# succinctlabs/tendermintx

Hardware: AMD Instinct MI355X
Metric: skip-circuit witness-gen ms at VALIDATOR_SET_SIZE_MAX=128 (lower is better)
Workload: dtype int64; 1 GPU; SkipCircuit VALIDATOR_SET_SIZE_MAX=128, batch of 256 proofs over 1 GPU(s) (BASELINE configs[3] batch per GPU, weak-scaled), 100 validators in 128 lanes, 4 distinct validator set(s) per batch, 90% sign; n_max=128, proofs_total=256, proofs_per_gpu=256, workload_name=survey8d, parallelism=proof-sharded x1, no data-path collective

## Files before the change

### include/tmx.h

```cpp
#ifndef TMX_H
#define TMX_H
#include <stddef.h>
#include <stdint.h>

#ifdef __cplusplus
extern "C" {
#endif

#define TMX_KIND_SKIP 0
#define TMX_KIND_STEP 1

#define TMX_N_MAX_LIMIT 512

#define TMX_VALIDATOR_MESSAGE_BYTES_LENGTH_MAX 124
#define TMX_VALIDATOR_BYTE_LENGTH_MAX 46
#define TMX_PROTOBUF_CHAIN_ID_SIZE_BYTES 52
#define TMX_HEADER_PROOF_DEPTH 4

#define TMX_FLAG_SIGNED 1u
#define TMX_FLAG_PRESENT 2u

typedef enum {
  TMX_OK = 0,
  TMX_ERR_BAD_ARG = -1,
// ... 235 lines not shown
int32_t tmx_finish_batch_device(tmx_ctx* ctx, int32_t kind, uint32_t n_proofs, const void* d_proofs, const void* d_targets,
                                const void* d_trusteds, const void* d_ed, void* d_out_elems, void* d_reports, void* hip_stream);
int32_t tmx_last_kernel_ms(tmx_ctx* ctx, float ms[TMX_N_KERNELS]);
int32_t tmx_kernel_ms_mean(tmx_ctx* ctx, uint32_t last_k, float ms[TMX_N_KERNELS]);
int32_t tmx_sync(tmx_ctx* ctx);
int32_t tmx_last_dedup(tmx_ctx* ctx, uint32_t* n_unique, uint32_t* used_tables);
enum tmx_proof_path {
  TMX_PROOF_PATH_NONE = 0,
  TMX_PROOF_PATH_TINY = 1,
  TMX_PROOF_PATH_ROLES = 2,
  TMX_PROOF_PATH_R168 = 3,
  TMX_PROOF_PATH_K256 = 4,
  TMX_PROOF_PATH_WIDE = 5
};
int32_t tmx_last_proof_path(tmx_ctx* ctx);

#define TMX_UNIQUE_ID_BYTES 128
void tmx_shard_range(uint64_t n_items, uint32_t rank, uint32_t world, uint64_t* lo, uint64_t* hi);
int32_t tmx_comm_unique_id(uint8_t out[TMX_UNIQUE_ID_BYTES]);
int32_t tmx_comm_create(tmx_ctx* ctx, const uint8_t unique_id[TMX_UNIQUE_ID_BYTES] , uint32_t rank, uint32_t world);
int32_t tmx_comm_destroy(tmx_ctx* ctx);
int32_t tmx_comm_info(const tmx_ctx* ctx, uint32_t* rank, uint32_t* world);
int32_t tmx_comm_abort(tmx_ctx* ctx);
int32_t tmx_comm_sync(tmx_ctx* ctx, void* hip_stream, uint32_t timeout_ms);
int32_t tmx_witness_batch_sharded_device(tmx_ctx* ctx, int32_t kind, uint32_t n_total, const void* d_proofs, const void* d_targets,
                                         const void* d_trusteds, void* d_out_elems, void* d_reports, uint32_t gather, void* hip_stream);
int32_t tmx_witness_validator_sharded_device(tmx_ctx* ctx, int32_t kind, uint32_t n_proofs, const void* d_proofs, const void* d_targets,
                                             const void* d_trusteds, void* d_out_elems, void* d_reports, void* hip_stream);

int32_t tmx_trace_rows_sharded_device(tmx_ctx* ctx, int32_t kind, uint32_t n_total, const void* d_targets, const void* d_trusteds, void* d_trace_out,
// ... 264 lines not shown
```

### tendermintx_amd/_lib.py

```python
import ctypes as C
import ctypes.util
import importlib.util
import os
import sys

_HERE = os.path.dirname(os.path.abspath(__file__))
LIB_PATH = os.environ.get("TMX_LIB") or os.path.join(_HERE, "libtmx.so")

KIND_SKIP, KIND_STEP = 0, 1
FLAG_SIGNED, FLAG_PRESENT = 1, 2
N_KERNELS = 4
KERNEL_NAMES = ("k_eddsa", "k_proof", "k_verdict", "k_serialize")
ED_STRIDE = 448
SEC_HINT, SEC_DERIVED, SEC_ALL = 1, 2, 3
PROOF_PATH_NONE, PROOF_PATH_TINY, PROOF_PATH_ROLES, PROOF_PATH_R168, PROOF_PATH_K256, PROOF_PATH_WIDE = range(6)
TRACE_LADDERS, TRACE_SHA512, TRACE_SHA256, TRACE_MATCH, TRACE_TREE, TRACE_HEADER, TRACE_ALL = 1, 2, 4, 8, 16, 32, 63
TRACE_LADDERS_QUOTIENT = 64
AIR_SHA256_HELPER_COLS, AIR_SHA256_CONSTRAINTS = 300, 315
TRACE_SHA256_HELPER, TRACE_SHA256_QUOTIENT = 128, 256
AIR_SHA256_SCHED_HELPER_COLS, AIR_SHA256_SCHED_CONSTRAINTS = 115, 117
TRACE_SHA256_SCHED_HELPER, TRACE_SHA256_SCHED_QUOTIENT = 512, 1024
AIR_SHA256_INIT_HELPER_COLS, AIR_SHA256_INIT_CONSTRAINTS = 315, 337
TRACE_SHA256_INIT_HELPER, TRACE_SHA256_INIT_QUOTIENT = 2048, 4096
TRACE_SHA256_LINK_HELPER, TRACE_SHA256_LINK_QUOTIENT = 8192, 16384
AIR_SHA256_PUBLIC_WIDTH, AIR_SHA256_LINK_HELPER_COLS, AIR_SHA256_LINK_CONSTRAINTS = 26, 33, 50


class ValidatorRec(C.Structure):
    _fields_ = [("pubkey", C.c_uint8 * 32), ("signature", C.c_uint8 * 64), ("message", C.c_uint8 * 124),
                ("message_byte_length", C.c_uint16), ("validator_byte_length", C.c_uint8), ("flags", C.c_uint8),
# ... 375 lines not shown
    L.tmx_witness_batch_sharded_device.argtypes = [C.c_void_p, C.c_int32, C.c_uint32, C.c_void_p, C.c_void_p, C.c_void_p, C.c_void_p, C.c_void_p,
                                                   C.c_uint32, C.c_void_p]
    L.tmx_witness_validator_sharded_device.argtypes = [C.c_void_p, C.c_int32, C.c_uint32, C.c_void_p, C.c_void_p, C.c_void_p, C.c_void_p, C.c_void_p,
                                                       C.c_void_p]
    L.tmx_trace_rows_sharded_device.argtypes = [C.c_void_p, C.c_int32, C.c_uint32, C.c_void_p, C.c_void_p, C.c_void_p, C.c_uint32, C.c_uint32, C.c_void_p]
    L.tmx_trace_rows_validator_sharded_device.argtypes = [C.c_void_p, C.c_int32, C.c_uint32, C.c_void_p, C.c_void_p, C.c_void_p, C.c_uint32, C.c_void_p]
    L.tmx_trace_commit_sharded_device.argtypes = [C.c_void_p, C.c_int32, C.c_uint32, C.c_uint32, C.c_uint32, C.c_uint32, C.c_void_p, C.c_void_p, C.c_void_p]
    L.tmx_last_kernel_ms.argtypes = [C.c_void_p, C.POINTER(C.c_float)]
    L.tmx_kernel_ms_mean.argtypes = [C.c_void_p, C.c_uint32, C.POINTER(C.c_float)]
    L.tmx_ctx_stream.restype = C.c_void_p
    L.tmx_ctx_stream.argtypes = [C.c_void_p]
    L.tmx_sync.argtypes = [C.c_void_p]
    L.tmx_last_dedup.argtypes = [C.c_void_p, C.POINTER(C.c_uint32), C.POINTER(C.c_uint32)]
    L.tmx_last_proof_path.restype = C.c_int32
    L.tmx_last_proof_path.argtypes = [C.c_void_p]
    L.tmx_key_cache_stats.argtypes = [C.c_void_p, C.POINTER(KeyCacheInfo)]
    L.tmx_key_cache_flush.argtypes = [C.c_void_p]
    L.tmx_key_cache_config.argtypes = [C.c_void_p, C.c_uint32, C.c_uint32]
    L.tmx_set_cache_stats.argtypes = [C.c_void_p, C.POINTER(C.c_uint32)]
    L.tmx_eddsa_lanes.argtypes = [C.c_void_p, C.c_uint32, C.c_void_p, C.c_void_p]
    L.tmx_skip_inputs_from_json.argtypes = [C.c_char_p, C.c_char_p, C.c_char_p, C.c_char_p, C.c_uint32, C.c_uint64,
                                            C.c_char_p, C.c_uint64, C.c_void_p, C.c_void_p, C.c_void_p]
    L.tmx_step_inputs_from_json.argtypes = [C.c_char_p, C.c_char_p, C.c_char_p, C.c_uint32, C.c_uint64, C.c_char_p,
                                            C.c_void_p, C.c_void_p]
    L.tmx_valid_skip_batch.argtypes = [C.c_void_p, C.c_uint32, C.c_void_p, C.c_uint32, C.c_void_p, C.c_void_p, C.c_void_p, C.c_void_p,
                                       C.c_void_p, C.c_void_p, C.c_void_p]
    L.tmx_skipcheck_inputs_from_json.argtypes = [C.c_char_p, C.c_char_p, C.c_char_p, C.c_uint32, C.c_void_p, C.POINTER(C.c_uint32), C.c_void_p,
                                                 C.POINTER(C.c_uint32), C.c_void_p, C.POINTER(C.c_uint32)]
    L.tmx_pack_skip_input.argtypes = [C.c_uint64, C.c_char_p, C.c_uint64, C.c_char_p]
    L.tmx_pack_skip_input.restype = None
# ... 20 lines not shown
```

### tendermintx_amd/context.py

```python
import ctypes as C

import numpy as np

from . import _lib
from ._lib import KIND_SKIP, KIND_STEP, Config, Report, check


def _indices(indices):
    if isinstance(indices, np.ndarray):
        return np.ascontiguousarray(indices.reshape(-1), dtype=np.uint64)
    return np.array([int(i) for i in indices], dtype=np.uint64)


class Context:

    def __init__(self, n_max, chain_id=b"celestia", skip_max=100800, device=0, max_batch=1):
        self._L = _lib.lib()
        self.n_max, self.chain_id, self.skip_max, self.max_batch = int(n_max), bytes(chain_id), int(skip_max), int(max_batch)
        cfg = Config()
        cfg.n_max = self.n_max
        cfg.chain_id_len = len(self.chain_id)
        for i, b in enumerate(self.chain_id[:52]):
            cfg.chain_id[i] = b
        cfg.skip_max = self.skip_max
# ... 524 lines not shown
        ms = (C.c_float * _lib.N_KERNELS)()
        check(self._L.tmx_kernel_ms_mean(self._h, last_k, ms), self._h)
        return dict(zip(_lib.KERNEL_NAMES, (float(x) for x in ms)))

    def last_dedup(self):
        u, t = C.c_uint32(), C.c_uint32()
        check(self._L.tmx_last_dedup(self._h, C.byref(u), C.byref(t)), self._h)
        return int(u.value), bool(t.value)

    def last_proof_path(self):
        path = int(self._L.tmx_last_proof_path(self._h))
        if path < 0:
            check(path, self._h)
        return path

    def key_cache_stats(self):
        info = _lib.KeyCacheInfo()
        check(self._L.tmx_key_cache_stats(self._h, C.byref(info)), self._h)
        return info.as_dict()

    def set_cache_stats(self):
        out = (C.c_uint32 * 8)()
        check(self._L.tmx_set_cache_stats(self._h, out), self._h)
        return dict(zip(("resident", "served", "computed", "inserted", "evicted", "capacity"), (int(x) for x in out)))

    def key_cache_flush(self):
        check(self._L.tmx_key_cache_flush(self._h), self._h)

    def key_cache_config(self, enabled=True, max_keys=0):
        check(self._L.tmx_key_cache_config(self._h, 1 if enabled else 0, int(max_keys)), self._h)
# ... 76 lines not shown
```

### tendermintx_amd/csrc/api.cpp

```cpp
#include <hip/hip_runtime_api.h>

#include <algorithm>
#include <chrono>
#include <cstdio>
#include <cstdlib>
#include <cstring>
#include <mutex>
#include <string>
#include <thread>
#include <vector>

#include "kernels.h"
#include "air.h"
#include "fri.h"
#include "ntt.h"
#include "poseidon.h"
#include "trace.h"
#include "tmx.h"
#include "value.h"

using namespace tmx;

static thread_local std::string g_tls_err;

// ... 244 lines not shown
  long tiny_max = -1;
  int one_launch_max = -1;
  bool proof_roles = true;
  int tail_wide = 1;
  int p1_early = -1;
  int hash_first = -1;
  bool walk_split = true;
  bool compact = true;
  bool set_cache = true;
  bool epi_late = true;
  bool ser_lanes = true;
  int fused_base = -1, fused_walk = -1;
  long inputs_first_min = -1;
  bool ser_rows = true;
  int writer_prio = -1;
  int tail_aside_min = -1;
  int few_wgs = 0;
  int tiny = -1;
};
static Knobs read_knobs() {
  Knobs k;
  const char* v;
  if ((v = std::getenv("TMX_DEDUP")) && v[0] >= '0' && v[0] <= '2') k.dedup_mode = (uint32_t)(v[0] - '0');
  k.key_cache = !((v = std::getenv("TMX_KEY_CACHE")) && v[0] == '0');
  if ((v = std::getenv("TMX_KEY_CACHE_KEYS")) && std::atoll(v) > 0) k.key_cache_keys = (uint32_t)std::min<long long>(std::atoll(v), 1 << 20);
  k.ser_split = !((v = std::getenv("TMX_SER_SPLIT")) && v[0] == '0');
  k.leaves = (v = std::getenv("TMX_LEAVES")) ? (v[0] != '0' ? 1 : 0) : -1;
  k.walk_parts = (v = std::getenv("TMX_WALK_PARTS")) ? (v[0] == '1' ? 1 : 0) : -1;
  k.ext_events = !((v = std::getenv("TMX_EXT_EVENTS")) && v[0] == '0');
  k.warm_schedule = (v = std::getenv("TMX_SCHEDULE")) ? (v[0] == 'w' ? 1 : 0) : -1;
  k.tiny = (v = std::getenv("TMX_TINY")) ? (v[0] != '0' ? 1 : 0) : -1;
  k.walk_split = !((v = std::getenv("TMX_WALK_SPLIT")) && v[0] == '0');
  k.proof_roles = !((v = std::getenv("TMX_PROOF_ROLES")) && v[0] == '0');
  if ((v = std::getenv("TMX_SER_ONE_LAUNCH"))) k.one_launch_max = std::atoi(v);
  if ((v = std::getenv("TMX_TINY_MAX"))) k.tiny_max = std::atol(v);
  if ((v = std::getenv("TMX_JOIN1"))) k.join1 = v[0] != '0';
  if ((v = std::getenv("TMX_PHASE1_MAX"))) k.phase1_max = std::atoi(v);
  k.hash_first = (v = std::getenv("TMX_HASH_FIRST")) ? (v[0] != '0' ? 1 : 0) : -1;
  if ((v = std::getenv("TMX_TAIL_WIDE"))) k.tail_wide = v[0] != '0' ? 1 : 0;
  k.p1_early = (v = std::getenv("TMX_P1_EARLY")) && v[0] >= '0' && v[0] <= '2' ? v[0] - '0' : -1;
  k.compact = !((v = std::getenv("TMX_COMPACT")) && v[0] == '0');
  k.set_cache = !((v = std::getenv("TMX_SET_CACHE")) && v[0] == '0');
  k.epi_late = !((v = std::getenv("TMX_EPI_LATE")) && v[0] == '0');
  if ((v = std::getenv("TMX_FEW_WGS"))) k.few_wgs = std::atoi(v);
  if ((v = std::getenv("TMX_TAIL_ASIDE_MIN"))) k.tail_aside_min = std::atoi(v);
  if ((v = std::getenv("TMX_WRITER_PRIO"))) k.writer_prio = std::atoi(v);
  k.ser_rows = !((v = std::getenv("TMX_SER_ROWS")) && v[0] == '0');
  if ((v = std::getenv("TMX_INPUTS_FIRST"))) k.inputs_first_min = std::atol(v);
  if ((v = std::getenv("TMX_FUSED_ROWS"))) {
    k.fused_base = std::atoi(v);
    const char* comma = std::strpbrk(v, ",:");
    k.fused_walk = comma ? std::atoi(comma + 1) : 0;
    if (k.fused_base < 0) k.fused_base = 0;
    if (k.fused_walk < 0) k.fused_walk = 0;
  }
  if ((v = std::getenv("TMX_SER_LANES"))) k.ser_lanes = std::atoi(v) != 0;
  return k;
}

struct tmx_ctx {
// ... 84 lines not shown
  void* d_air6 = nullptr;
  size_t air6_bytes = 0;
  void* d_deepv = nullptr;
  size_t deepv_bytes = 0;
  struct IdxSlot { uint64_t* h = nullptr; uint64_t* d = nullptr; uint64_t cap = 0; hipEvent_t ev = nullptr; bool used = false; };
  static constexpr int IDX_RING = 4;
  IdxSlot idx_ring[IDX_RING];
  uint32_t idx_next = 0;
  void* comm = nullptr;
  bool comm_aborted = false;
  uint32_t comm_rank = 0, comm_world = 1;
  void* d_tiny = nullptr;
  void* d_shadow = nullptr;
  bool slot_tiny[EV_RING_DECL] = {};
  uint64_t last_lanes = 0;
  int32_t last_proof_path = TMX_PROOF_PATH_NONE;
  void *d_ed = nullptr, *d_tl = nullptr, *d_lr = nullptr, *d_pf = nullptr, *d_nodes_t = nullptr, *d_nodes_r = nullptr, *d_reports = nullptr;
  void *d_in_proofs = nullptr, *d_in_targets = nullptr, *d_in_trusteds = nullptr, *d_out = nullptr;
  uint64_t d_out_elems = 0;
  hipEvent_t ev_trace[17] = {};
  hipEvent_t ev_trace_rest[2] = {};
  void* d_trace_tmp = nullptr;
  void* d_pack = nullptr;
  void* d_val_lut[2] = {nullptr, nullptr};
  void* d_value = nullptr;
  uint64_t d_value_bytes = 0;
  uint64_t d_pack_bytes = 0;
  uint32_t sections = 3;
  void* d_ntt_w[TMX_NTT_MAX_LOG + 1] = {};
  void* d_ntt_m[2][TMX_NTT_MAX_LOG + 1] = {};
// ... 178 lines not shown
  if (st) { (void)late_epilogue(); return st; }
  if (defer3 && (st0 = side3_inputs())) { (void)late_epilogue(); return st0; }
  if ((st0 = late_epilogue())) return st0;
  if (leaves_first) {
    if (!c->ev_hash_recorded) HIPCK(c, hipEventRecord(c->ev_hash, s));
    HIPCK(c, hipStreamWaitEvent(c->side3, c->ev_hash, 0));
    if ((st0 = serialize(prog.mask_p1, c->side3, beside_chain_wgs))) return st0;
    HIPCK(c, hipEventRecord(c->ev_join3, c->side3));
  }
  const bool tail_aside = tail_aside_early;
  const bool small_tail = K.ser_split && !tail_aside;
  if (small_tail && !leaves_first) {
    if (!c->ev_hash_recorded) HIPCK(c, hipEventRecord(c->ev_hash, s));
    HIPCK(c, hipStreamWaitEvent(c->side, c->ev_hash, 0));
  }
  st0 = K.ser_split ? serialize(prog.mask_proof | (leaves_first ? 0u : prog.mask_leaves) | (small_tail && !leaves_first ? prog.mask_p1 : 0u), c->side) : TMX_OK;
  if (st0) return st0;
  if (!roles && c->setc.table && (rc = launch_setc_evict(c->setc, c->setc_epoch, c->side)))
    return fail(c, TMX_ERR_HIP, std::string("k_setc_evict launch: ") + hipGetErrorString((hipError_t)rc));
  const bool p1_early = leaves_first || small_tail ||
                        (K.ser_split && c->ev_hash_recorded && (K.p1_early >= 0 ? K.p1_early != 0 : throughput));
  if (p1_early && !leaves_first && !small_tail) {
    HIPCK(c, hipStreamWaitEvent(c->side, c->ev_hash, 0));
    if ((st0 = serialize(prog.mask_p1, c->side, K.p1_early == 2 ? 0u : beside_chain_wgs))) return st0;
  }

  HIPCK(c, hipStreamWaitEvent(c->side, c->ev_join3, 0));
  HIPCK(c, hipEventRecord(c->ev_join, c->side));
  if (!c->fin_done_attached) HIPCK(c, hipEventRecord(ev[1], s));
  if (small_tail) {
    if (fin_split && K.join1) {
      HIPCK(c, hipStreamWaitEvent(c->side2, evs[1], 0));
      HIPCK(c, hipEventRecord(c->ev_direct, c->side2));
      HIPCK(c, hipStreamWaitEvent(s, c->ev_direct, 0));
    } else {
      HIPCK(c, hipStreamWaitEvent(s, evs[1], 0));
      if (fin_split) HIPCK(c, hipStreamWaitEvent(s, c->ev_direct, 0));
    }
    const bool xv = K.ext_events && n_proofs != 0;
    if (!xv) HIPCK(c, hipEventRecord(evs[2], s));
    const bool with_rows = d_out_elems != nullptr;
    uint32_t tail_mask = (mask_final | prog.mask_tail) & (((c->sections & TMX_SEC_HINT) ? prog.mask_hint : 0u) | ((c->sections & TMX_SEC_DERIVED) ? prog.mask_derived : 0u) | (1u << 31));
    if (K.tail_wide && !(tail_mask & mask_final))
      rc = launch_verdict_tail_wide((uint32_t)kind, n, n_proofs, tl + TL_OFF_ED, TL_STRIDE, c->d_pf, reports, row, prog.sp, src, c->d_lut[kind], c->d_wave_sec[kind],
                                    c->d_seams[kind], (uint32_t)prog.seam_waves.size(), with_rows ? d_out_elems : nullptr, tail_mask, prog.tail_dep_elem, s,
                                    xv ? evs[2] : nullptr, xv ? evs[3] : nullptr);
    else
    rc = launch_verdict_tail((uint32_t)kind, n, n_proofs, tl + TL_OFF_ED, TL_STRIDE, c->d_pf, reports, row, prog.sp, src, c->d_lut[kind], c->d_seams[kind],
                             (uint32_t)prog.seam_waves.size(), with_rows ? d_out_elems : nullptr, tail_mask, s, xv ? evs[2] : nullptr, xv ? evs[3] : nullptr);
    if (rc) return fail(c, TMX_ERR_HIP, std::string("k_verdict_tail launch: ") + hipGetErrorString((hipError_t)rc));
    if (!xv) HIPCK(c, hipEventRecord(evs[3], s));
    HIPCK(c, hipStreamWaitEvent(s, c->ev_join, 0));
  } else if (K.ser_split) {
    if (K.join1) {
      HIPCK(c, hipStreamWaitEvent(c->side2, evs[1], 0));
      HIPCK(c, hipStreamWaitEvent(c->side2, ev[1], 0));
    } else {
    HIPCK(c, hipStreamWaitEvent(c->side2, ev[1], 0));
    HIPCK(c, hipStreamWaitEvent(c->side2, evs[1], 0));
    }
    if (K.tail_wide && n_proofs) {
      const bool xv = K.ext_events;
      if (!xv) HIPCK(c, hipEventRecord(evs[2], c->side2));
      const uint32_t tail_mask = prog.mask_tail & (((c->sections & TMX_SEC_HINT) ? prog.mask_hint : 0u) | ((c->sections & TMX_SEC_DERIVED) ? prog.mask_derived : 0u) | (1u << 31));
      rc = launch_verdict_tail_wide((uint32_t)kind, n, n_proofs, tl + TL_OFF_ED, TL_STRIDE, c->d_pf, reports, row, prog.sp, src, c->d_lut[kind], c->d_wave_sec[kind],
                                    c->d_seams[kind], (uint32_t)prog.seam_waves.size(), d_out_elems, tail_mask, prog.tail_dep_elem, c->side2,
                                    xv ? evs[2] : nullptr, xv ? evs[3] : nullptr);
// ... 1 lines not shown
      if (!xv) HIPCK(c, hipEventRecord(evs[3], c->side2));
    } else {
    HIPCK(c, hipEventRecord(evs[2], c->side2));
    rc = launch_verdict((uint32_t)kind, n, n_proofs, tl + TL_OFF_ED, TL_STRIDE, c->d_pf, reports, row, c->side2);
    if (rc) return fail(c, TMX_ERR_HIP, std::string("k_verdict launch: ") + hipGetErrorString((hipError_t)rc));
    HIPCK(c, hipEventRecord(evs[3], c->side2));
    if ((st0 = serialize(prog.mask_tail, c->side2))) return st0;
    }
    HIPCK(c, hipStreamWaitEvent(c->side2, c->ev_join, 0));
    HIPCK(c, hipEventRecord(c->ev_tail, c->side2));
    if (mask_final | (p1_early ? 0u : prog.mask_p1)) {
      HIPCK(c, hipStreamWaitEvent(s, evs[1], 0));
      if ((st0 = serialize(mask_final | (p1_early ? 0u : prog.mask_p1), s))) return st0;
    }
    HIPCK(c, hipStreamWaitEvent(s, c->ev_tail, 0));
  } else {
    HIPCK(c, hipStreamWaitEvent(s, c->ev_join, 0));
    if (fin_split) HIPCK(c, hipStreamWaitEvent(s, c->ev_direct, 0));
    HIPCK(c, hipEventRecord(evs[2], s));
    rc = launch_verdict((uint32_t)kind, n, n_proofs, tl + TL_OFF_ED, TL_STRIDE, c->d_pf, reports, row, s);
    if (rc) return fail(c, TMX_ERR_HIP, std::string("k_verdict launch: ") + hipGetErrorString((hipError_t)rc));
    HIPCK(c, hipEventRecord(evs[3], s));
    HIPCK(c, hipEventRecord(ev[2], s));
    if ((st0 = serialize(prog.mask_inputs | prog.mask_proof | prog.mask_leaves | mask_final | prog.mask_p1 | prog.mask_tail, s))) return st0;
  }
  HIPCK(c, hipEventRecord(ev[3], s));
  c->slot_tiny[slot] = false;
  c->last_stream = s; c->last_stream_valid = true;
  c->ev_done = ev[3];
  c->last_kind = kind; c->last_n_proofs = n_proofs;
  c->n_calls++;
// ... 86 lines not shown
  }
  T.mask_inputs = prog.mask_inputs & want;
  T.mask_after = (prog.mask_proof | prog.mask_leaves | prog.mask_p1 | (T.row.rows ? 0u : prog.mask_final)) & want;
  T.mask_tail = prog.mask_tail & want;
  T.tail_dep_elem = prog.tail_dep_elem;
  const bool x = K.ext_events;
  if (!x) HIPCK(c, hipEventRecord(ev[0], s));
  int rc = launch_tiny(T, s, x ? ev[0] : nullptr, x ? ev[1] : nullptr);
  if (rc) return fail(c, TMX_ERR_HIP, std::string("k_tiny launch: ") + hipGetErrorString((hipError_t)rc));
  if (!x) { HIPCK(c, hipEventRecord(ev[1], s)); HIPCK(c, hipEventRecord(ev[2], s)); }
  rc = launch_tiny_tail(T, s, x ? ev[2] : nullptr, x ? ev[3] : nullptr);
  if (rc) return fail(c, TMX_ERR_HIP, std::string("k_tiny_tail launch: ") + hipGetErrorString((hipError_t)rc));
  if (!x) HIPCK(c, hipEventRecord(ev[3], s));
  if ((st = tiny_key_pipeline(c, n_proofs * n, ev[1]))) return st;
  c->last_proof_path = TMX_PROOF_PATH_TINY;
  c->slot_tiny[slot] = true;
  c->last_stream = s; c->last_stream_valid = true;
  c->ev_done = ev[3];
  c->last_kind = kind; c->last_n_proofs = n_proofs;
  c->n_calls++;
  return TMX_OK;
}

static int32_t check_batch_args(tmx_ctx* c, int32_t kind, uint32_t n_proofs, const void* d_proofs, const void* d_targets, const void* d_trusteds) {
  if (!c || (kind != TMX_KIND_SKIP && kind != TMX_KIND_STEP) || !d_proofs || !d_targets) return TMX_ERR_BAD_ARG;
  if (kind == TMX_KIND_SKIP && !d_trusteds) return fail(c, TMX_ERR_BAD_ARG, "skip needs the trusted hash fields");
  if (n_proofs > c->cfg.max_batch) return fail(c, TMX_ERR_CAPACITY, "n_proofs exceeds the context's max_batch");
  return TMX_OK;
}

// ... 545 lines not shown
}

int32_t tmx_last_dedup(tmx_ctx* c, uint32_t* n_unique, uint32_t* used_tables) {
  if (!c || !n_unique || !used_tables) return TMX_ERR_BAD_ARG;
  *n_unique = 0; *used_tables = 0;
  if (c->last_lanes == 0) return TMX_OK;
  uint32_t st[KC_STATE_WORDS];
  int32_t r = read_kc_state(c, st);
  if (r) return r;
  *n_unique = st[KC_LAST_NEW] + st[KC_LAST_HIT_KEYS];
  *used_tables = (c->knobs.dedup_mode != 0 && (st[KC_LAST_HIT_LANES] != 0 || (st[KC_LAST_BUILT] != 0 && st[KC_LAST_USE_NEW] != 0))) ? 1u : 0u;
  return TMX_OK;
}

int32_t tmx_last_proof_path(tmx_ctx* c) { return c ? c->last_proof_path : TMX_ERR_BAD_ARG; }

int32_t tmx_key_cache_stats(tmx_ctx* c, tmx_key_cache_info* out) {
  if (!c || !out) return TMX_ERR_BAD_ARG;
  uint32_t st[KC_STATE_WORDS];
  int32_t r = read_kc_state(c, st);
  if (r) return r;
  uint64_t tot[8];
  std::memcpy(tot, st + KC_TOTALS, sizeof(uint64_t) * 6);
  std::memset(out, 0, sizeof *out);
  out->capacity_keys = c->kc.cap; out->resident_keys = st[KC_RESIDENT]; out->enabled = c->kc.persist; out->epoch = st[KC_EPOCH];
  out->bytes_per_key = keytab_bytes_per_key() + key_bytes_per_key() + 32;
  out->last_new_keys = st[KC_LAST_NEW]; out->last_hit_keys = st[KC_LAST_HIT_KEYS]; out->last_hit_lanes = st[KC_LAST_HIT_LANES];
  out->last_built_keys = st[KC_LAST_BUILT];
  out->hit_lanes = tot[KC_TOT_HIT_LANES]; out->miss_lanes = tot[KC_TOT_MISS_LANES]; out->built_keys = tot[KC_TOT_BUILT];
  out->evicted_keys = tot[KC_TOT_EVICTED]; out->evictions = tot[KC_TOT_GC_RUNS]; out->launches = tot[KC_TOT_LAUNCHES];
// ... 3400 lines not shown
```

### tendermintx_amd/csrc/kernels.h

```cpp
#pragma once
#include <stddef.h>
#include <stdint.h>

#include "layout.h"

namespace tmx {

struct KeyCache {
  uint32_t cap;
  uint32_t hash_mask;
  uint32_t new_cap;
  uint32_t persist;
  uint32_t* d_hash;
  uint32_t* d_pk;
  uint32_t* d_used;
  uint32_t* d_free;
  uint32_t* d_state;
  uint32_t* hint;
};
enum : uint32_t { KC_FREE_HEAD = 0, KC_N_FREE = 1, KC_EPOCH = 2, KC_RESIDENT = 3, KC_LAST_NEW = 4, KC_LAST_HIT_KEYS = 5, KC_LAST_HIT_LANES = 6,
                  KC_LAST_BUILT = 7, KC_LAST_USE_NEW = 8, KC_TOTALS = 16 , KC_STATE_WORDS = 32 };
enum : uint32_t { KC_TOT_HIT_LANES = 0, KC_TOT_MISS_LANES = 1, KC_TOT_BUILT = 2, KC_TOT_EVICTED = 3, KC_TOT_GC_RUNS = 4, KC_TOT_LAUNCHES = 5 };

size_t base_table_bytes();
// ... 48 lines not shown
                 void* done = nullptr, const SetCache& SC = SetCache{});
constexpr uint32_t KC_EPILOGUE_CLEARS_UP_TO = 1u << 16;
int launch_leaves(uint32_t kind, uint32_t n, uint32_t n_proofs, const void* d_target, const void* d_trusted, void* d_lt, uint32_t lt_stride, void* d_lr,
                  void* stream, void* done = nullptr);
int launch_valid_skip(uint32_t n_cand, uint32_t n_max, const void* d_start, uint32_t n_start, const void* d_targets, const void* d_nt, const void* d_sigs,
                      const void* d_ns, void* d_valid, void* d_shared, void* d_total, void* stream);
int launch_verdict(uint32_t kind, uint32_t n, uint32_t n_proofs, const void* d_ed, uint32_t ed_stride, void* d_pf, void* d_reports, const RowOut& row,
                   void* stream, void* started = nullptr, void* done = nullptr);
int launch_verdict_tail(uint32_t kind, uint32_t n, uint32_t n_proofs, const void* d_ed, uint32_t ed_stride, void* d_pf, void* d_reports, const RowOut& row,
                        const SerializeProgram& S, const SerializeSources& src, const void* d_lut, const void* d_seam_waves, uint32_t n_seams, void* d_out,
                        uint32_t sec_mask, void* stream, void* started = nullptr, void* done = nullptr);
int launch_verdict_tail_wide(uint32_t kind, uint32_t n, uint32_t n_proofs, const void* d_ed, uint32_t ed_stride, void* d_pf, void* d_reports,
                             const RowOut& row, const SerializeProgram& S, const SerializeSources& src, const void* d_lut, const void* d_wave_sec,
                             const void* d_seam_waves, uint32_t n_seams, void* d_out, uint32_t sec_mask, uint32_t tail_dep_elem, void* stream,
                             void* started = nullptr, void* done = nullptr);
int launch_setc_evict(const SetCache& SC, uint32_t epoch, void* stream);
SerializeProgram resolve_serialize_program(const SerializeProgram& S, const SerializeSources& src);
int launch_serialize_claim(const SerializeProgram& S_resolved, const FusedRows& F, void* d_zero_ctr, void* stream, uint32_t max_wgs);
int launch_serialize(const SerializeProgram& S, const SerializeSources& src, const void* d_lut, const void* d_wave_sec, const void* d_seam_waves,
                     uint32_t n_seams, uint32_t n_proofs, void* d_out, uint32_t sec_mask, void* stream, uint32_t max_wgs = 0, uint32_t proof0 = 0);
int launch_pack_rows(const void* d_rows, void* d_out, uint32_t elem_stride, uint32_t first, uint32_t row_elems, uint32_t n_proofs, bool as_u32,
                     void* stream);


constexpr uint32_t TINY_MAX_LANES = 2048;
struct TinyLaunch {
  uint32_t n_lanes;
  const void* d_target;
  void* d_ed;
  uint32_t ed_stride;
// ... 30 lines not shown
```

### tendermintx_amd/csrc/kernels.hip

```cpp
#include "kernels.h"

#include <hip/hip_runtime.h>
#include <hip/hip_ext.h>
#include <cstdlib>
#include <cstring>

#include <type_traits>

#include "ge25519.hpp"
#include "inv25519.hpp"
#include "fe16.hpp"
#include "winv25519.hpp"
#include "sc25519.hpp"
#include "sha2.hpp"

namespace tmx {

__device__ __forceinline__ uint32_t bswap32(uint32_t x) { return __builtin_bswap32(x); }
__device__ __forceinline__ uint32_t ld32(const uint8_t* p) { return *reinterpret_cast<const uint32_t*>(p); }
__device__ __forceinline__ uint64_t ld64(const uint8_t* p) { return *reinterpret_cast<const uint64_t*>(p); }
__device__ __forceinline__ void st32(uint8_t* p, uint32_t v) { *reinterpret_cast<uint32_t*>(p) = v; }
__device__ __forceinline__ void st64(uint8_t* p, uint64_t v) { *reinterpret_cast<uint64_t*>(p) = v; }

#ifdef TMX_WAVE_PROF
// ... 1960 lines not shown
  ProofParams P, const uint8_t *__restrict__ in_proof, const uint8_t *__restrict__ in_target, const uint8_t *__restrict__ in_trusted,  \
      uint8_t *__restrict__ lt, uint32_t lt_stride, uint8_t *__restrict__ lr, uint8_t *__restrict__ pf_all,                          \
      uint8_t *__restrict__ nodes_t_all, uint8_t *__restrict__ nodes_r_all, uint8_t *__restrict__ reports, SetCache SC
__global__ __launch_bounds__(PROOF_THREADS) void k_proof(TMX_PROOF_ARGS) {
  proof_body<256>(P, in_proof, in_target, in_trusted, lt, lt_stride, lr, pf_all, nodes_t_all, nodes_r_all, reports, SC);
}
__global__ __launch_bounds__(PROOF_THREADS) __attribute__((amdgpu_waves_per_eu(3, 3))) void k_proof_r168(TMX_PROOF_ARGS) {
  proof_body<128>(P, in_proof, in_target, in_trusted, lt, lt_stride, lr, pf_all, nodes_t_all, nodes_r_all, reports, SC);
}
__global__ __launch_bounds__(PROOF_THREADS_WIDE) void k_proof_wide(TMX_PROOF_ARGS) {
  proof_body<TMX_N_LIMIT>(P, in_proof, in_target, in_trusted, lt, lt_stride, lr, pf_all, nodes_t_all, nodes_r_all, reports, SC);
}
#undef TMX_PROOF_ARGS


__device__ __forceinline__ void verdict_body(uint32_t kind, uint32_t n, const uint8_t* __restrict__ ed, uint32_t ed_stride,
                                             uint8_t* __restrict__ pf_all, uint8_t* __restrict__ reports, const RowOut& rowout) {
  const uint32_t p = blockIdx.x, t = threadIdx.x;
  const uint8_t* edp = ed + (size_t)p * n * ed_stride;
  uint32_t first_bad = 0xffffffffu;
  for (uint32_t i = t; i < n; i += 64)
    if (ld32(edp + (size_t)i * ed_stride + ED_OFF_OK) == 0) first_bad = first_bad < i ? first_bad : i;
  if (rowout.rows) {
    for (uint32_t i = t; i < n; i += 64) {
      const uint8_t* lt = edp + (size_t)i * ed_stride + (TL_OFF_LT - TL_OFF_ED);
      uint64_t* row = row_d1b(rowout, p * n + i) + D1B_ED_ELEMS;
      const uint32_t f0 = ld32(lt + LN_OFF_FLAGS), f1 = ld32(lt + LN_OFF_FLAGS + 4);
      row[0] = f0 & 0xff; row[1] = (f0 >> 8) & 0xff; row[2] = (f0 >> 16) & 0xff; row[3] = f0 >> 24; row[4] = f1 & 0xff; row[5] = (f1 >> 8) & 0xff;
      row[6] = ld32(lt + LN_OFF_TOT); row[7] = ld32(lt + LN_OFF_TOT + 4); row[8] = ld32(lt + LN_OFF_ACC); row[9] = ld32(lt + LN_OFF_ACC + 4);
    }
  }
#pragma unroll
  for (int off = 32; off > 0; off >>= 1) {
    uint32_t o = __shfl_xor(first_bad, off);
    first_bad = first_bad < o ? first_bad : o;
  }
  if (t == 0 && first_bad != 0xffffffffu) {
    const uint32_t idx = kind == 0 ? 9u : 7u;
    uint8_t* pf = pf_all + (size_t)p * PF_STRIDE;
    uint8_t* rp = reports + (size_t)p * 64;
    st32(pf + PF_OFF_CHECKS + 4 * idx, 0u);
    st32(pf + PF_OFF_ALLOK, 0u);
    st32(rp + 32, 0u);
    st32(rp + 36, ld32(rp + 36) | (1u << idx));
    st32(rp + 40, first_bad);
  }
// ... 326 lines not shown
      const uint32_t sp = SA.seam_waves[i / S.span], e = sp * S.span + i % S.span;
      if (sp < SA.tail_first_span && e < S.elem_stride) row[e] = e < S.elem_count ? serialize_one(S.sec[section_of(S, e)], SA.lut, proof, e) : 0;
    }
    return;
  }
  const uint32_t proof = b;
  if (threadIdx.x < 64) verdict_body(kind, n, ed, ed_stride, pf_all, reports, rowout);
  __builtin_amdgcn_fence(__ATOMIC_SEQ_CST, "workgroup");
  __syncthreads();
  if (!SA.out) return;
  uint64_t* row = SA.out + (size_t)proof * S.elem_stride;
  for (uint32_t e = SA.tail_first_span * S.span + threadIdx.x; e < S.elem_stride; e += T)
    if (SA.tail_mask || SA.wave_sec[e / S.span] == 0xffu) row[e] = e < S.elem_count ? serialize_one(S.sec[section_of(S, e)], SA.lut, proof, e) : 0;
}

static inline hipStream_t S_(void* s) { return reinterpret_cast<hipStream_t>(s); }
static inline hipEvent_t E_(void* e) { return reinterpret_cast<hipEvent_t>(e); }

constexpr int BASE_W = 13;
constexpr uint32_t BASE_ENTRIES = BaseWin<BASE_W>::ENTRIES;
__global__ __launch_bounds__(64) void k_selftest_f16(uint32_t n, uint32_t d, const uint32_t* __restrict__ in, uint32_t* __restrict__ out) {
  const uint32_t i = blockIdx.x, tid = threadIdx.x;
  if (i >= n) return;
  const f16::Ctx c = f16::make_ctx((int)tid);
  const uint32_t a = in[128 * i + tid], b = in[128 * i + 64 + tid];
  out[256 * i + tid] = f16::mul(a, b, c);
  uint32_t Q = a, V = f16::with_xy(a, c);
  for (uint32_t k = 0; k < d; k++) V = f16::dbl(V, Q, c);
  out[256 * i + 64 + tid] = Q;
  if (tid < 4) {
// ... 402 lines not shown
}
int launch_verdict_tail_wide(uint32_t kind, uint32_t n, uint32_t n_proofs, const void* d_ed, uint32_t ed_stride, void* d_pf, void* d_reports,
                             const RowOut& row, const SerializeProgram& S0, const SerializeSources& src, const void* d_lut, const void* d_wave_sec,
                             const void* d_seam_waves, uint32_t n_seams, void* d_out, uint32_t sec_mask, uint32_t tail_dep_elem, void* stream, void* started,
                             void* done) {
  if (n_proofs == 0) return 0;
  TinyLaunch T;
  std::memset(&T, 0, sizeof T);
  T.S = &S0; T.src = &src; T.d_lut = d_lut; T.d_wave_sec = d_wave_sec; T.d_seams = d_seam_waves; T.n_seams = n_seams; T.d_out = d_out;
  const TinySer SA = tiny_ser(T, sec_mask & 0x7fffffffu, sec_mask, tail_dep_elem);
  const uint32_t total = n_proofs + (SA.out ? n_proofs * (1 + SA.n_blocks) : 0u);
  hipExtLaunchKernelGGL(k_verdict_tail_wide, dim3(total), dim3(TAIL_WIDE_THREADS), 0, S_(stream), E_(started), E_(done), 0, kind, n, n_proofs,
                        reinterpret_cast<const uint8_t*>(d_ed), ed_stride, reinterpret_cast<uint8_t*>(d_pf), reinterpret_cast<uint8_t*>(d_reports), row, SA);
  return (int)hipGetLastError();
}

}

#ifdef TMX_WAVE_PROF
extern "C" int tmx_debug_wave_prof(uint32_t* out, uint32_t cap_records, uint32_t* n_out, int reset) {
  uint32_t n = 0;
  hipError_t e = hipMemcpyFromSymbol(&n, HIP_SYMBOL(tmx::g_wave_prof_n), 4);
  if (e != hipSuccess) return (int)e;
  if (n > tmx::WAVE_PROF_CAP) n = tmx::WAVE_PROF_CAP;
  if (n > cap_records) n = cap_records;
  if (out && n && (e = hipMemcpyFromSymbol(out, HIP_SYMBOL(tmx::g_wave_prof), (size_t)n * 32)) != hipSuccess) return (int)e;
  if (n_out) *n_out = n;
  if (reset) { const uint32_t z = 0; if ((e = hipMemcpyToSymbol(HIP_SYMBOL(tmx::g_wave_prof_n), &z, 4)) != hipSuccess) return (int)e; }
  return 0;
}
// ... 2 lines not shown
```

Before: 1.378 us.

## Split wide verdict tail into independent side-stream part and dependent verdict part

Splits the wide verdict tail into two kernels. One runs on a secondary stream as soon as the eddsa results are ready and writes the per-proof row words plus every serialize seam that does not depend on final or p1 sections. The other runs on the main stream after the proof kernel and computes the verdict plus the dependent seams and tail spans. In throughput mode p1 serialization is also moved early, aiming to take work off the critical path after the proof stage, at the cost of extra launches and events. A tail-form query API is added for introspection.

```diff
diff --git a/include/tmx.h b/include/tmx.h
--- a/include/tmx.h
+++ b/include/tmx.h
@@ -273,6 +273,15 @@
   TMX_PROOF_PATH_WIDE = 5
 };
 int32_t tmx_last_proof_path(tmx_ctx* ctx);
+enum tmx_tail_form {
+  TMX_TAIL_FORM_NONE = 0,
+  TMX_TAIL_FORM_TINY = 1,
+  TMX_TAIL_FORM_SMALL = 2,
+  TMX_TAIL_FORM_ASIDE = 3,
+  TMX_TAIL_FORM_SPLIT = 4,
+  TMX_TAIL_FORM_LAUNCHES = 5
+};
+int32_t tmx_last_tail_form(tmx_ctx* ctx);
 
 #define TMX_UNIQUE_ID_BYTES 128
 void tmx_shard_range(uint64_t n_items, uint32_t rank, uint32_t world, uint64_t* lo, uint64_t* hi);
diff --git a/tendermintx_amd/_lib.py b/tendermintx_amd/_lib.py
--- a/tendermintx_amd/_lib.py
+++ b/tendermintx_amd/_lib.py
@@ -14,6 +14,7 @@
 ED_STRIDE = 448
 SEC_HINT, SEC_DERIVED, SEC_ALL = 1, 2, 3
 PROOF_PATH_NONE, PROOF_PATH_TINY, PROOF_PATH_ROLES, PROOF_PATH_R168, PROOF_PATH_K256, PROOF_PATH_WIDE = range(6)
+TAIL_FORM_NONE, TAIL_FORM_TINY, TAIL_FORM_SMALL, TAIL_FORM_ASIDE, TAIL_FORM_SPLIT, TAIL_FORM_LAUNCHES = range(6)
 TRACE_LADDERS, TRACE_SHA512, TRACE_SHA256, TRACE_MATCH, TRACE_TREE, TRACE_HEADER, TRACE_ALL = 1, 2, 4, 8, 16, 32, 63
 TRACE_LADDERS_QUOTIENT = 64
 AIR_SHA256_HELPER_COLS, AIR_SHA256_CONSTRAINTS = 300, 315
@@ -419,6 +420,8 @@
     L.tmx_last_dedup.argtypes = [C.c_void_p, C.POINTER(C.c_uint32), C.POINTER(C.c_uint32)]
     L.tmx_last_proof_path.restype = C.c_int32
     L.tmx_last_proof_path.argtypes = [C.c_void_p]
+    L.tmx_last_tail_form.restype = C.c_int32
+    L.tmx_last_tail_form.argtypes = [C.c_void_p]
     L.tmx_key_cache_stats.argtypes = [C.c_void_p, C.POINTER(KeyCacheInfo)]
     L.tmx_key_cache_flush.argtypes = [C.c_void_p]
     L.tmx_key_cache_config.argtypes = [C.c_void_p, C.c_uint32, C.c_uint32]
diff --git a/tendermintx_amd/context.py b/tendermintx_amd/context.py
--- a/tendermintx_amd/context.py
+++ b/tendermintx_amd/context.py
@@ -562,6 +562,12 @@
             check(path, self._h)
         return path
 
+    def last_tail_form(self):
+        form = int(self._L.tmx_last_tail_form(self._h))
+        if form < 0:
+            check(form, self._h)
+        return form
+
     def key_cache_stats(self):
         info = _lib.KeyCacheInfo()
         check(self._L.tmx_key_cache_stats(self._h, C.byref(info)), self._h)
diff --git a/tendermintx_amd/csrc/api.cpp b/tendermintx_amd/csrc/api.cpp
--- a/tendermintx_amd/csrc/api.cpp
+++ b/tendermintx_amd/csrc/api.cpp
@@ -282,6 +282,7 @@
   long inputs_first_min = -1;
   bool ser_rows = true;
   int writer_prio = -1;
+  int tail_split = -1;
   int tail_aside_min = -1;
   int few_wgs = 0;
   int tiny = -1;
@@ -312,6 +313,7 @@
   k.epi_late = !((v = std::getenv("TMX_EPI_LATE")) && v[0] == '0');
   if ((v = std::getenv("TMX_FEW_WGS"))) k.few_wgs = std::atoi(v);
   if ((v = std::getenv("TMX_TAIL_ASIDE_MIN"))) k.tail_aside_min = std::atoi(v);
+  k.tail_split = (v = std::getenv("TMX_TAIL_SPLIT")) ? (v[0] != '0' ? 1 : 0) : -1;
   if ((v = std::getenv("TMX_WRITER_PRIO"))) k.writer_prio = std::atoi(v);
   k.ser_rows = !((v = std::getenv("TMX_SER_ROWS")) && v[0] == '0');
   if ((v = std::getenv("TMX_INPUTS_FIRST"))) k.inputs_first_min = std::atol(v);
@@ -426,6 +428,7 @@
   void* d_shadow = nullptr;
   bool slot_tiny[EV_RING_DECL] = {};
   uint64_t last_lanes = 0;
+  int32_t last_tail_form = TMX_TAIL_FORM_NONE;
   int32_t last_proof_path = TMX_PROOF_PATH_NONE;
   void *d_ed = nullptr, *d_tl = nullptr, *d_lr = nullptr, *d_pf = nullptr, *d_nodes_t = nullptr, *d_nodes_r = nullptr, *d_reports = nullptr;
   void *d_in_proofs = nullptr, *d_in_targets = nullptr, *d_in_trusteds = nullptr, *d_out = nullptr;
@@ -634,15 +637,29 @@
     if (!c->ev_hash_recorded) HIPCK(c, hipEventRecord(c->ev_hash, s));
     HIPCK(c, hipStreamWaitEvent(c->side, c->ev_hash, 0));
   }
+  const bool tail_split = tail_aside && K.tail_wide && n_proofs != 0 && (K.tail_split >= 0 ? K.tail_split != 0 : throughput);
+  const uint32_t tail_sel = prog.mask_tail & (((c->sections & TMX_SEC_HINT) ? prog.mask_hint : 0u) | ((c->sections & TMX_SEC_DERIVED) ? prog.mask_derived : 0u) | (1u << 31));
+  const uint32_t tail_dep_mask = prog.mask_final | prog.mask_p1;
+  if (tail_split) {
+    HIPCK(c, hipStreamWaitEvent(c->side2, evs[1], 0));
+    if (fin_split && K.join1) HIPCK(c, hipEventRecord(c->ev_direct, c->side2));
+    rc = launch_tail_indep(n, n_proofs, tl + TL_OFF_ED, TL_STRIDE, row, prog.sp, src, c->d_lut[kind], c->d_wave_sec[kind], c->d_seams[kind],
+                           (uint32_t)prog.seam_waves.size(), d_out_elems, tail_sel, tail_dep_mask, prog.tail_dep_elem, c->side2);
+    if (rc) return fail(c, TMX_ERR_HIP, std::string("k_tail_indep launch: ") + hipGetErrorString((hipError_t)rc));
+    if (!roles && c->setc.table && (rc = launch_setc_evict(c->setc, c->setc_epoch, c->side2)))
+      return fail(c, TMX_ERR_HIP, std::string("k_setc_evict launch: ") + hipGetErrorString((hipError_t)rc));
+    HIPCK(c, hipEventRecord(c->ev_tail, c->side2));
+  }
   st0 = K.ser_split ? serialize(prog.mask_proof | (leaves_first ? 0u : prog.mask_leaves) | (small_tail && !leaves_first ? prog.mask_p1 : 0u), c->side) : TMX_OK;
   if (st0) return st0;
-  if (!roles && c->setc.table && (rc = launch_setc_evict(c->setc, c->setc_epoch, c->side)))
+  if (!tail_split && !roles && c->setc.table && (rc = launch_setc_evict(c->setc, c->setc_epoch, c->side)))
     return fail(c, TMX_ERR_HIP, std::string("k_setc_evict launch: ") + hipGetErrorString((hipError_t)rc));
   const bool p1_early = leaves_first || small_tail ||
-                        (K.ser_split && c->ev_hash_recorded && (K.p1_early >= 0 ? K.p1_early != 0 : throughput));
+                        (K.ser_split && c->ev_hash_recorded && (K.p1_early >= 0 ? K.p1_early != 0 : (throughput || tail_split)));
   if (p1_early && !leaves_first && !small_tail) {
     HIPCK(c, hipStreamWaitEvent(c->side, c->ev_hash, 0));
-    if ((st0 = serialize(prog.mask_p1, c->side, K.p1_early == 2 ? 0u : beside_chain_wgs))) return st0;
+    const bool full_grid = K.p1_early >= 0 ? K.p1_early == 2 : !throughput;
+    if ((st0 = serialize(prog.mask_p1, c->side, full_grid ? 0u : beside_chain_wgs))) return st0;
   }
 
   HIPCK(c, hipStreamWaitEvent(c->side, c->ev_join3, 0));
@@ -671,6 +688,27 @@
     if (rc) return fail(c, TMX_ERR_HIP, std::string("k_verdict_tail launch: ") + hipGetErrorString((hipError_t)rc));
     if (!xv) HIPCK(c, hipEventRecord(evs[3], s));
     HIPCK(c, hipStreamWaitEvent(s, c->ev_join, 0));
+    c->last_tail_form = TMX_TAIL_FORM_SMALL;
+  } else if (tail_split) {
+    if (fin_split && K.join1) {
+      HIPCK(c, hipStreamWaitEvent(s, c->ev_direct, 0));
+    } else {
+      HIPCK(c, hipStreamWaitEvent(s, evs[1], 0));
+      if (fin_split) HIPCK(c, hipStreamWaitEvent(s, c->ev_direct, 0));
+    }
+    const bool xv = K.ext_events;
+    if (!xv) HIPCK(c, hipEventRecord(evs[2], s));
+    rc = launch_verdict_dep((uint32_t)kind, n, n_proofs, tl + TL_OFF_ED, TL_STRIDE, c->d_pf, reports, prog.sp, src, c->d_lut[kind], c->d_wave_sec[kind],
+                            c->d_seams[kind], (uint32_t)prog.seam_waves.size(), d_out_elems, tail_sel, tail_dep_mask, prog.tail_dep_elem, s,
+                            xv ? evs[2] : nullptr, xv ? evs[3] : nullptr);
+    if (rc) return fail(c, TMX_ERR_HIP, std::string("k_verdict_dep launch: ") + hipGetErrorString((hipError_t)rc));
+    if (!xv) HIPCK(c, hipEventRecord(evs[3], s));
+    if (mask_final | (p1_early ? 0u : prog.mask_p1)) {
+      if ((st0 = serialize(mask_final | (p1_early ? 0u : prog.mask_p1), s))) return st0;
+    }
+    HIPCK(c, hipStreamWaitEvent(s, c->ev_tail, 0));
+    HIPCK(c, hipStreamWaitEvent(s, c->ev_join, 0));
+    c->last_tail_form = TMX_TAIL_FORM_SPLIT;
   } else if (K.ser_split) {
     if (K.join1) {
       HIPCK(c, hipStreamWaitEvent(c->side2, evs[1], 0));
@@ -702,7 +740,9 @@
       if ((st0 = serialize(mask_final | (p1_early ? 0u : prog.mask_p1), s))) return st0;
     }
     HIPCK(c, hipStreamWaitEvent(s, c->ev_tail, 0));
+    c->last_tail_form = K.tail_wide && n_proofs ? TMX_TAIL_FORM_ASIDE : TMX_TAIL_FORM_LAUNCHES;
   } else {
+    c->last_tail_form = TMX_TAIL_FORM_LAUNCHES;
     HIPCK(c, hipStreamWaitEvent(s, c->ev_join, 0));
     if (fin_split) HIPCK(c, hipStreamWaitEvent(s, c->ev_direct, 0));
     HIPCK(c, hipEventRecord(evs[2], s));
@@ -819,6 +859,7 @@
   if (!x) HIPCK(c, hipEventRecord(ev[3], s));
   if ((st = tiny_key_pipeline(c, n_proofs * n, ev[1]))) return st;
   c->last_proof_path = TMX_PROOF_PATH_TINY;
+  c->last_tail_form = TMX_TAIL_FORM_TINY;
   c->slot_tiny[slot] = true;
   c->last_stream = s; c->last_stream_valid = true;
   c->ev_done = ev[3];
@@ -1394,6 +1435,7 @@
 }
 
 int32_t tmx_last_proof_path(tmx_ctx* c) { return c ? c->last_proof_path : TMX_ERR_BAD_ARG; }
+int32_t tmx_last_tail_form(tmx_ctx* c) { return c ? c->last_tail_form : TMX_ERR_BAD_ARG; }
 
 int32_t tmx_key_cache_stats(tmx_ctx* c, tmx_key_cache_info* out) {
   if (!c || !out) return TMX_ERR_BAD_ARG;
diff --git a/tendermintx_amd/csrc/kernels.h b/tendermintx_amd/csrc/kernels.h
--- a/tendermintx_amd/csrc/kernels.h
+++ b/tendermintx_amd/csrc/kernels.h
@@ -86,6 +86,13 @@
                              const RowOut& row, const SerializeProgram& S, const SerializeSources& src, const void* d_lut, const void* d_wave_sec,
                              const void* d_seam_waves, uint32_t n_seams, void* d_out, uint32_t sec_mask, uint32_t tail_dep_elem, void* stream,
                              void* started = nullptr, void* done = nullptr);
+int launch_tail_indep(uint32_t n, uint32_t n_proofs, const void* d_ed, uint32_t ed_stride, const RowOut& row, const SerializeProgram& S,
+                      const SerializeSources& src, const void* d_lut, const void* d_wave_sec, const void* d_seam_waves, uint32_t n_seams, void* d_out,
+                      uint32_t sec_mask, uint32_t dep_mask, uint32_t tail_dep_elem, void* stream);
+int launch_verdict_dep(uint32_t kind, uint32_t n, uint32_t n_proofs, const void* d_ed, uint32_t ed_stride, void* d_pf, void* d_reports,
+                       const SerializeProgram& S, const SerializeSources& src, const void* d_lut, const void* d_wave_sec, const void* d_seam_waves,
+                       uint32_t n_seams, void* d_out, uint32_t sec_mask, uint32_t dep_mask, uint32_t tail_dep_elem, void* stream,
+                       void* started = nullptr, void* done = nullptr);
 int launch_setc_evict(const SetCache& SC, uint32_t epoch, void* stream);
 SerializeProgram resolve_serialize_program(const SerializeProgram& S, const SerializeSources& src);
 int launch_serialize_claim(const SerializeProgram& S_resolved, const FusedRows& F, void* d_zero_ctr, void* stream, uint32_t max_wgs);
diff --git a/tendermintx_amd/csrc/kernels.hip b/tendermintx_amd/csrc/kernels.hip
--- a/tendermintx_amd/csrc/kernels.hip
+++ b/tendermintx_amd/csrc/kernels.hip
@@ -1998,6 +1998,17 @@
 #undef TMX_PROOF_ARGS
 
 
+__device__ __forceinline__ void d1b_proof_words(uint32_t n, const uint8_t* __restrict__ ed, uint32_t ed_stride, const RowOut& rowout, uint32_t p,
+                                                uint32_t t, uint32_t step) {
+  const uint8_t* edp = ed + (size_t)p * n * ed_stride;
+  for (uint32_t i = t; i < n; i += step) {
+    const uint8_t* lt = edp + (size_t)i * ed_stride + (TL_OFF_LT - TL_OFF_ED);
+    uint64_t* row = row_d1b(rowout, p * n + i) + D1B_ED_ELEMS;
+    const uint32_t f0 = ld32(lt + LN_OFF_FLAGS), f1 = ld32(lt + LN_OFF_FLAGS + 4);
+    row[0] = f0 & 0xff; row[1] = (f0 >> 8) & 0xff; row[2] = (f0 >> 16) & 0xff; row[3] = f0 >> 24; row[4] = f1 & 0xff; row[5] = (f1 >> 8) & 0xff;
+    row[6] = ld32(lt + LN_OFF_TOT); row[7] = ld32(lt + LN_OFF_TOT + 4); row[8] = ld32(lt + LN_OFF_ACC); row[9] = ld32(lt + LN_OFF_ACC + 4);
+  }
+}
 __device__ __forceinline__ void verdict_body(uint32_t kind, uint32_t n, const uint8_t* __restrict__ ed, uint32_t ed_stride,
                                              uint8_t* __restrict__ pf_all, uint8_t* __restrict__ reports, const RowOut& rowout) {
   const uint32_t p = blockIdx.x, t = threadIdx.x;
@@ -2005,15 +2016,7 @@
   uint32_t first_bad = 0xffffffffu;
   for (uint32_t i = t; i < n; i += 64)
     if (ld32(edp + (size_t)i * ed_stride + ED_OFF_OK) == 0) first_bad = first_bad < i ? first_bad : i;
-  if (rowout.rows) {
-    for (uint32_t i = t; i < n; i += 64) {
-      const uint8_t* lt = edp + (size_t)i * ed_stride + (TL_OFF_LT - TL_OFF_ED);
-      uint64_t* row = row_d1b(rowout, p * n + i) + D1B_ED_ELEMS;
-      const uint32_t f0 = ld32(lt + LN_OFF_FLAGS), f1 = ld32(lt + LN_OFF_FLAGS + 4);
-      row[0] = f0 & 0xff; row[1] = (f0 >> 8) & 0xff; row[2] = (f0 >> 16) & 0xff; row[3] = f0 >> 24; row[4] = f1 & 0xff; row[5] = (f1 >> 8) & 0xff;
-      row[6] = ld32(lt + LN_OFF_TOT); row[7] = ld32(lt + LN_OFF_TOT + 4); row[8] = ld32(lt + LN_OFF_ACC); row[9] = ld32(lt + LN_OFF_ACC + 4);
-    }
-  }
+  if (rowout.rows) d1b_proof_words(n, ed, ed_stride, rowout, p, t, 64);
 #pragma unroll
   for (int off = 32; off > 0; off >>= 1) {
     uint32_t o = __shfl_xor(first_bad, off);
@@ -2370,6 +2373,63 @@
     if (SA.tail_mask || SA.wave_sec[e / S.span] == 0xffu) row[e] = e < S.elem_count ? serialize_one(S.sec[section_of(S, e)], SA.lut, proof, e) : 0;
 }
 
+__device__ __forceinline__ bool seam_waits(const SerializeProgram& S, uint32_t sp, uint32_t dep_mask, uint32_t tail_first_span) {
+  const uint32_t lo = sp * S.span;
+  if (sp >= tail_first_span || lo >= S.elem_count) return true;
+  const uint32_t hi = lo + S.span < S.elem_count ? lo + S.span - 1 : S.elem_count - 1;
+  for (int k = section_of(S, lo), last = section_of(S, hi); k <= last; k++)
+    if ((dep_mask >> k) & 1u) return true;
+  return false;
+}
+__device__ __forceinline__ void tail_seams(const TinySer& SA, uint32_t proof, uint32_t dep_mask, bool want_dep) {
+  const SerializeProgram& S = SA.S;
+  uint64_t* row = SA.out + (size_t)proof * S.elem_stride;
+  const uint32_t waves = blockDim.x >> 6, lane = threadIdx.x & 63u;
+  for (uint32_t j = threadIdx.x >> 6; j < SA.n_seams; j += waves) {
+    const uint32_t sp = __builtin_amdgcn_readfirstlane(SA.seam_waves[j]);
+    if (sp >= SA.tail_first_span || seam_waits(S, sp, dep_mask, SA.tail_first_span) != want_dep) continue;
+#pragma unroll 4
+    for (uint32_t e = sp * S.span + lane; e < (sp + 1) * S.span; e += 64)
+      if (e < S.elem_stride) row[e] = e < S.elem_count ? serialize_one(S.sec[section_of(S, e)], SA.lut, proof, e) : 0;
+  }
+}
+__global__ __launch_bounds__(TAIL_WIDE_THREADS) void k_tail_indep(uint32_t n, uint32_t n_proofs, const uint8_t* __restrict__ ed, uint32_t ed_stride,
+                                                                  RowOut rowout, TinySer SA, uint32_t dep_mask) {
+  const uint32_t b = blockIdx.x, T = blockDim.x;
+  const SerializeProgram& S = SA.S;
+  __builtin_amdgcn_s_setprio(3);
+  if (b >= n_proofs) {
+    if (!SA.out) return;
+    const uint32_t per = SA.n_blocks;
+    const uint32_t r = b - n_proofs, proof = r / per, k = r - proof * per;
+    const uint32_t span = __builtin_amdgcn_readfirstlane((SA.first_block + k) * 4 + (threadIdx.x >> 6));
+    if (span < SA.tail_first_span) serialize_span<SER_SPAN_ELEMS>(S, SA.lut, SA.wave_sec, SA.out, SA.mask, proof, span);
+    return;
+  }
+  const uint32_t proof = b;
+  if (rowout.rows) d1b_proof_words(n, ed, ed_stride, rowout, proof, threadIdx.x, T);
+  if (SA.out) tail_seams(SA, proof, dep_mask, false);
+}
+__global__ __launch_bounds__(TAIL_WIDE_THREADS) void k_verdict_dep(uint32_t kind, uint32_t n, const uint8_t* __restrict__ ed, uint32_t ed_stride,
+                                                                   uint8_t* __restrict__ pf_all, uint8_t* __restrict__ reports, TinySer SA,
+                                                                   uint32_t dep_mask, uint32_t n_proofs) {
+  const uint32_t T = blockDim.x;
+  const SerializeProgram& S = SA.S;
+  __builtin_amdgcn_s_setprio(3);
+  if (blockIdx.x >= n_proofs) {
+    if (SA.out) tail_seams(SA, blockIdx.x - n_proofs, dep_mask, true);
+    return;
+  }
+  const uint32_t proof = blockIdx.x;
+  if (threadIdx.x < 64) verdict_body(kind, n, ed, ed_stride, pf_all, reports, RowOut{});
+  __builtin_amdgcn_fence(__ATOMIC_SEQ_CST, "workgroup");
+  __syncthreads();
+  if (!SA.out) return;
+  uint64_t* row = SA.out + (size_t)proof * S.elem_stride;
+  for (uint32_t e = SA.tail_first_span * S.span + threadIdx.x; e < S.elem_stride; e += T)
+    if (SA.tail_mask || SA.wave_sec[e / S.span] == 0xffu) row[e] = e < S.elem_count ? serialize_one(S.sec[section_of(S, e)], SA.lut, proof, e) : 0;
+}
+
 static inline hipStream_t S_(void* s) { return reinterpret_cast<hipStream_t>(s); }
 static inline hipEvent_t E_(void* e) { return reinterpret_cast<hipEvent_t>(e); }
 
@@ -2802,6 +2862,34 @@
                         reinterpret_cast<const uint8_t*>(d_ed), ed_stride, reinterpret_cast<uint8_t*>(d_pf), reinterpret_cast<uint8_t*>(d_reports), row, SA);
   return (int)hipGetLastError();
 }
+static TinySer tail_ser(const SerializeProgram& S0, const SerializeSources& src, const void* d_lut, const void* d_wave_sec, const void* d_seam_waves,
+                        uint32_t n_seams, void* d_out, uint32_t sec_mask, uint32_t tail_dep_elem) {
+  TinyLaunch T;
+  std::memset(&T, 0, sizeof T);
+  T.S = &S0; T.src = &src; T.d_lut = d_lut; T.d_wave_sec = d_wave_sec; T.d_seams = d_seam_waves; T.n_seams = n_seams; T.d_out = d_out;
+  return tiny_ser(T, sec_mask & 0x7fffffffu, sec_mask, tail_dep_elem);
+}
+int launch_tail_indep(uint32_t n, uint32_t n_proofs, const void* d_ed, uint32_t ed_stride, const RowOut& row, const SerializeProgram& S0,
+                      const SerializeSources& src, const void* d_lut, const void* d_wave_sec, const void* d_seam_waves, uint32_t n_seams, void* d_out,
+                      uint32_t sec_mask, uint32_t dep_mask, uint32_t tail_dep_elem, void* stream) {
+  if (n_proofs == 0 || (!d_out && !row.rows)) return 0;
+  const TinySer SA = tail_ser(S0, src, d_lut, d_wave_sec, d_seam_waves, n_seams, d_out, sec_mask, tail_dep_elem);
+  const uint32_t total = n_proofs * (1 + (SA.out ? SA.n_blocks : 0u));
+  hipLaunchKernelGGL(k_tail_indep, dim3(total), dim3(TAIL_WIDE_THREADS), 0, S_(stream), n, n_proofs, reinterpret_cast<const uint8_t*>(d_ed), ed_stride, row,
+                     SA, dep_mask);
+  return (int)hipGetLastError();
+}
+int launch_verdict_dep(uint32_t kind, uint32_t n, uint32_t n_proofs, const void* d_ed, uint32_t ed_stride, void* d_pf, void* d_reports,
+                       const SerializeProgram& S0, const SerializeSources& src, const void* d_lut, const void* d_wave_sec, const void* d_seam_waves,
+                       uint32_t n_seams, void* d_out, uint32_t sec_mask, uint32_t dep_mask, uint32_t tail_dep_elem, void* stream, void* started,
+                       void* done) {
+  if (n_proofs == 0) return 0;
+  const TinySer SA = tail_ser(S0, src, d_lut, d_wave_sec, d_seam_waves, n_seams, d_out, sec_mask, tail_dep_elem);
+  hipExtLaunchKernelGGL(k_verdict_dep, dim3(n_proofs * (SA.out ? 2u : 1u)), dim3(TAIL_WIDE_THREADS), 0, S_(stream), E_(started), E_(done), 0, kind, n,
+                        reinterpret_cast<const uint8_t*>(d_ed), ed_stride, reinterpret_cast<uint8_t*>(d_pf), reinterpret_cast<uint8_t*>(d_reports), SA,
+                        dep_mask, n_proofs);
+  return (int)hipGetLastError();
+}
 
 }
 
```

New measurement: 1.448 us. 1.05x slower.
